# NLESC-JCER/Fortran_Davidson

Hardware: AMD Instinct MI355X
Metric: Davidson iterations/sec (dense DPR solve, matrix resident in HBM) + A*V HBM GB/s vs roofline (higher is better)
Workload: dtype f64

## Files before the change

fortran_davidson_amd/csrc/engine.hip:

```cpp
#include "engine_internal.h"

thread_local std::string g_err;
int fail(const std::string& msg) {
  g_err = msg;
  return 1;
}

int bind(E* e) {
  e->h0_take = e->h0_cols;
  e->h0_cols = 0;
  HIPCHK(hipSetDevice(e->device));
  return 0;
}

int collect_events(E* e) {
  e->ev_open = 0;
  for (int i = 0; i < e->ev_used; ++i) {
    if (!e->ev_done[i]) continue;
    HIPCHK(hipEventSynchronize(e->ev[i][1]));
    float ms = 0;
    HIPCHK(hipEventElapsedTime(&ms, e->ev[i][0], e->ev[i][1]));
    if (e->ev_kind[i] == 0) {
      e->st.apply_ms += ms;
      e->st.apply_bytes += e->ev_bytes[i];
// ... 146 lines not shown
}

Tune tune_from_env() {
  Tune t;
  auto geti = [](const char* name, int dflt) { const char* ev = getenv(name); return ev && *ev ? atoi(ev) : dflt; };
  t.sym_wide = geti("DAV_SYM_WIDE", t.sym_wide);
  t.sym_wide32 = geti("DAV_SYM_WIDE32", t.sym_wide32);
  t.sym_pair = geti("DAV_SYM_PAIR", t.sym_pair);
  t.sym_quad = geti("DAV_SYM_QUAD", t.sym_quad);
  t.sym_overlap = geti("DAV_SYM_OVERLAP", t.sym_overlap);
  t.sym_r = geti("DAV_SYM_R", t.sym_r);
  t.sym_tall = geti("DAV_SYM_TALL", t.sym_tall);
  t.sym_gen_wide = geti("DAV_SYM_GEN_WIDE", 1);
  t.sym_run = std::max(0, geti("DAV_SYM_RUN", 0));
  t.sym_run9 = std::max(0, geti("DAV_SYM_RUN9", 0));
  t.sym_mfma4 = geti("DAV_SYM_MFMA4", t.sym_mfma4);
  t.mv_target = std::max(0, geti("DAV_MV_TARGET", 0));
  t.mv_nsplit = std::max(0, geti("DAV_MV_NSPLIT", 0));
  t.b_resident = geti("DAV_B_RESIDENT", t.b_resident);
  t.coll_direct = geti("DAV_COLL_DIRECT", t.coll_direct);
  t.pg_pin = geti("DAV_PG_PIN", t.pg_pin);
  t.gram_wgs = geti("DAV_GRAM_WGS", t.gram_wgs);
  gram_set_fuse_chunks(geti("DAV_GRAM_FUSE", 0));
  t.gjd_trace = getenv("DAV_GJD_TRACE") != nullptr;
  t.harness_libm = geti("DAV_HARNESS_LIBM", 0);
  t.no_h0 = geti("DAV_NO_H0", 0);
  t.coll_select = geti("DAV_COLL_SELECT", 1);
  t.coll_trial_corrupt = geti("DAV_COLL_TRIAL_CORRUPT", 0);
  t.coll_forced = getenv("DAV_SYM_OVERLAP") != nullptr || getenv("DAV_COLL_DIRECT") != nullptr;
  return t;
// ... 456 lines not shown
```

fortran_davidson_amd/csrc/engine_apply.hip:

```cpp
#include "engine_internal.h"

bool inner_f32_tiles(E* e, OpDesc& o) {
  if (e->inner_bits != 32 || o.kind != DAV_KIND_DENSE || o.storage != 1 || o.a32_refused) return false;
  if (o.a32_valid) return true;
  const size_t count = (size_t)std::max<int64_t>(e->sym.ntiles, 1) * SYM_TB * SYM_TB;
  if (!o.a32 && pool_malloc(&o.a32, sizeof(float) * count) != hipSuccess) {
    (void)hipGetLastError();
    o.a32 = nullptr;
    o.a32_refused = true;
    return false;
  }
  launch_tiles_to_f32(e->stream, o.a, o.a32, (int64_t)count);
  o.a32_valid = true;
  return true;
}

static double* sym_slab_t(const E* e, const SymLaunch& L) { return e->sym_slab + (int64_t)L.ngroups * L.dstride; }
static void sym_sweep(E* e, const SymLaunch& L, const OpDesc& o, const SymSet& set, const double* xt) {
  if (L.nitems == 0) return;
  const SymPlan* pl = L.plan;
  const void* tiles = L.use32 ? (const void*)o.a32 : (const void*)o.a;
  double *slabD = e->sym_slab, *slabT = sym_slab_t(e, L);
  const int64_t xs = e->xt_group_stride, ds = L.dstride, ts = L.tstride;
  switch (L.family) {
    case SYM_ROW_STORED:
      return launch_matvec_sym(e->stream, o.a, set.row_off, set.items, set.nitems, xt, L.kk, slabD, slabT, L.ngroups, xs, ds, ts);
    case SYM_ROW_GENERATED:
      return launch_matvec_sym_generated(e->stream, op_params(o), e->n, set.items, set.nitems, xt, L.kk, slabD, slabT, L.ngroups, xs, ds, ts);
    case SYM_SUPER:
      return launch_matvec_sym9(e->stream, L.R, o.kind != DAV_KIND_DENSE, tiles, L.use32, set.row_off, o.kind != DAV_KIND_DENSE ? op_params(o) : OpParams{},
                                e->n, e->sym_nb, pl->items, pl->nitems, pl->zslot_begin, xt, L.kk, slabD, slabT, L.nwg, xs, ds, ts, e->tune.sym_mfma4 != 0);
    case SYM_WIDE:
    case SYM_WIDE_F32:
      return launch_matvec_symw(e->stream, L.nbw, L.tall, L.use32, tiles, set.row_off, e->sym_nb, pl->items, pl->nitems, pl->zslot_begin, xt, L.kk, slabD, slabT, L.nwg, xs, ds, ts);
    case SYM_WIDE_GENERATED:
      return launch_matvec_symw_generated(e->stream, op_params(o), e->n, e->sym_nb, pl->items, pl->nitems, pl->zslot_begin, xt, L.kk, slabD, slabT, L.nwg, xs, ds, ts);
  }
}

static void count_apply(E* e, int which, int kk) { if (which == DAV_OP_A) { e->st.applies += 1; e->st.apply_cols += kk; } }

static int pack_operand(E* e, const double* src, int kk, bool gather) {
  launch_pack_xt(e->stream, src, e->ldp, e->nloc, e->nslab, kk, e->xt, e->xt_group_stride, e->row0);
  if (!gather) return 0;
  const int ngroups = (kk + 15) / 16;
  CollGroup grp(e);
  CHK(grp.begin(5, 8.0 * (double)e->nslab * 16 * ngroups * e->nranks));
  for (int g = 0; g < ngroups; ++g)
    CHK(coll_allgather(e, e->xt + g * e->xt_group_stride + e->row0 * 16, e->xt + g * e->xt_group_stride, (size_t)e->nslab * 16));
  return grp.end("all-gather of the new block", e->stream);
}

static void sym_reduce_groups(E* e, const SymLaunch& L, const SymSet& set, const int64_t* owned, double* out, int64_t chunk_rows, bool accumulate) {
  const int64_t total_rows = (int64_t)e->nranks * e->nslab;
  const double* slabT = sym_slab_t(e, L);
  for (int g = 0; g < L.ngroups; ++g) {
    const int kg = std::min(16, L.kk - 16 * g);
    const double *d = e->sym_slab + g * L.dstride, *t = slabT + g * L.tstride;
    double* og = out + (size_t)g * 16 * (size_t)(chunk_rows ? total_rows : e->ldp);
    if (L.plan)
      launch_sym9_reduce(e->stream, d, t, L.plan->row_begin, L.plan->zslot_begin, owned, L.plan->next_owned, L.R, e->sym_nb, e->nloc, kg, og, e->ldp,
                         chunk_rows, total_rows, accumulate);
    else
      launch_sym_reduce(e->stream, d, t, set.row_begin, owned, e->sym_nb, e->nloc, kg, og, e->ldp, chunk_rows, total_rows, accumulate);
  }
}

static int ensure_sym_wpart(E* e) {
  if (e->sym_wpart) return 0;
  HIPCHK(pool_malloc(&e->sym_wpart, sizeof(double) * (size_t)e->nranks * (size_t)e->nslab * 64));
  HIPCHK(pool_malloc(&e->sym_wrecv, sizeof(double) * (size_t)e->nslab * 64));
  return 0;
}

static int sym_scatter_to_panel(E* e, int kk, double* dst, bool accumulate, const char* what, double* h0 = nullptr, size_t h0_count = 0) {
// ... 541 lines not shown
```

fortran_davidson_amd/csrc/engine_internal.h:

```cpp
#pragma once
#include "davidson_hip_private.h"
#include "kernels.h"
#include "ingest.h"

#include <dlfcn.h>
#include <fcntl.h>
#include <pthread.h>
#include <sys/mman.h>
#include <sys/stat.h>
#include <unistd.h>
#include <rccl/rccl.h>

#include <algorithm>
#include <chrono>
#include <condition_variable>
#include <ctime>
#include <mutex>
#include <cmath>
#include <cstdio>
#include <cstring>
#include <numeric>
#include <string>
#include <thread>
#include <vector>
// ... 51 lines not shown
  do {                                                                                             \
    ncclResult_t r_ = (call);                                                                      \
    if (r_ != ncclSuccess) return fail(std::string(#call) + " failed: " + g_rccl.GetErrorString(r_)); \
  } while (0)

struct LocalGroup;
struct ShmGroup;

struct SymPlan {
  int R = 0, nitems = 0, nsuper = 0;
  int64_t zslots = 0;
  int* items = nullptr;
  int* row_begin = nullptr;
  int* zslot_begin = nullptr;
  int* next_owned = nullptr;
};
struct SymSet {
  std::vector<int64_t> row_off_h;
  int64_t* row_off = nullptr;
  int64_t ntiles = 0;
  int nitems = 0;
  int* items = nullptr;
  int* row_begin = nullptr;
  SymPlan plan[2];
  bool built = false;
};
void sym_set_release(SymSet& s);
enum SymFamily { SYM_ROW_STORED, SYM_ROW_GENERATED, SYM_SUPER, SYM_WIDE, SYM_WIDE_GENERATED, SYM_WIDE_F32 };
struct SymLaunch {
  SymFamily family = SYM_SUPER;
  int kk = 0, ngroups = 0;
  int R = 0, nwg = 0, nbw = 1;
  bool use32 = false, tall = false;
  const SymPlan* plan = nullptr;
  int nitems = 0;
  int64_t dstride = 0, tstride = 0;
  int gen_evals = 0;
};

// ... 55 lines not shown

constexpr int N_SMALL = 4;
constexpr int N_EVPAIRS = 64;

struct Tune {
  int sym_wide = 2;
  int sym_wide32 = 1;
  int sym_pair = 1;
  int sym_quad = 1;
  int sym_overlap = 0;
  int sym_r = 0;
  int sym_tall = 1;
  int sym_gen_wide = 1;
  int sym_run = 0;
  int sym_run9 = 0;
  int sym_mfma4 = 1;
  int64_t mv_target = 0;
  int64_t mv_nsplit = 0;
  int gram_wgs = 0;
  int pg_pin = 1;
  int coll_direct = 0;
  int b_resident = 1;
  bool gjd_trace = false;
  int coll_select = 1;
  int coll_trial_corrupt = 0;
  bool coll_forced = false;
  int no_h0 = 0;
  int harness_libm = 0;
};
Tune tune_from_env();
// ... 220 lines not shown
```

fortran_davidson_amd/csrc/engine_operators.hip:

```cpp
#include "engine_internal.h"

int refresh_diag_host(E* e, int which) {
  if (which == DAV_OP_A) e->basis_order.clear();
  std::vector<double>& d = e->diag_host[which];
  d.assign((size_t)e->n, 0.0);
  if (!has_comm(e)) {
    CHK(need_comm(e));
    HIPCHK(hipMemcpyAsync(d.data(), e->op[which].diag, sizeof(double) * e->n, hipMemcpyDeviceToHost, e->stream));
    HIPCHK(hipStreamSynchronize(e->stream));
  } else {
    CHK(coll_allgather(e, e->op[which].diag, e->gather_dev, (size_t)e->nslab));
    HIPCHK(hipMemcpyAsync(d.data(), e->gather_dev, sizeof(double) * e->n, hipMemcpyDeviceToHost, e->stream));
    HIPCHK(hipStreamSynchronize(e->stream));
  }
  return 0;
}

static bool sym_wide_enabled(const E* e) { return e->tune.sym_wide > 1; }

static int sym_schedule(const E* e, int kk, bool stored_fp64) {
  const int forced = e->tune.sym_r;
  const int nb = (int)(e->ncols_pad / SYM_TB);
  int R = nb >= 200 ? (kk <= 8 ? 4 : 2) : (nb >= 64 && stored_fp64 ? 2 : 1);
  const bool tall = stored_fp64 && kk > 8 && kk <= 16 && nb >= 200 && sym_wide_enabled(e) && e->tune.sym_tall != 0;
// ... 9 lines not shown
  const bool stored = o.kind == DAV_KIND_DENSE;
  const int wide = e->tune.sym_wide;
  if (R == 0) {
    R = sym_schedule(e, kk, stored && !use32);
    if (use32 && R == 1) R = 2;
  }
  SymLaunch L;
  L.kk = kk; L.ngroups = L.nwg = (kk + 15) / 16; L.use32 = use32; L.R = R;
  if (R == 1) {
    L.family = stored ? SYM_ROW_STORED : SYM_ROW_GENERATED;
    L.nitems = set.nitems;
    L.dstride = (int64_t)set.nitems * 16 * SYM_TB;
    L.tstride = (int64_t)e->sym_nb * (e->sym_nb - 1) / 2 * 16 * SYM_TB;
  } else {
    L.plan = &set.plan[R == 4 ? 1 : 0];
    L.nitems = L.plan->nitems;
    L.dstride = (int64_t)L.nitems * R * 16 * SYM_TB;
    L.tstride = L.plan->zslots * 16 * SYM_TB;
    if (stored && !use32 && wide > 0 && ((R == 2 && (kk > 16 || wide > 1)) || (R == 4 && kk > 8 && kk <= 16))) {
      L.family = SYM_WIDE; L.nbw = kk > 16 ? 2 : 1; L.tall = R == 4;
    } else if (generated_polynomial(o) && R == 2 && kk > 16 && wide > 0 && e->tune.sym_gen_wide) {
      L.family = SYM_WIDE_GENERATED; L.nbw = 2;
    } else if (stored && use32 && wide > 1 && e->tune.sym_wide32 && R == 2 && kk <= 16) {
      L.family = SYM_WIDE_F32;
    }
    L.nwg = (L.ngroups + L.nbw - 1) / L.nbw;
  }
  L.gen_evals = stored ? 0 : L.nwg;
  return L;
}

std::vector<int> sym_group_owners(int nb, int nranks) {
  const int ng = (nb + 3) / 4;
  std::vector<int> owner(ng, 0);
  std::vector<int64_t> load(nranks, 0);
  for (int q = ng - 1; q >= 0; --q) {
    int64_t tiles = 0;
    for (int I = 4 * q; I < std::min(nb, 4 * q + 4); ++I) tiles += I + 1;
    int best = 0;
    for (int r = 1; r < nranks; ++r)
      if (load[r] < load[best]) best = r;
    owner[q] = best;
    load[best] += tiles;
  }
  return owner;
}

void sym_set_release(SymSet& s) {
  pool_free(s.row_off); pool_free(s.items); pool_free(s.row_begin);
  for (SymPlan& pl : s.plan) { pool_free(pl.items); pool_free(pl.row_begin); pool_free(pl.zslot_begin); pool_free(pl.next_owned); }
  s = SymSet();
}

int sym_setup(E* e) {
  if (e->sym.built) return 0;
  const int nb = (int)(e->ncols_pad / SYM_TB);
  e->sym_nb = nb;
  return sym_build_set(e, 0, nb, e->sym);
}

int sym_build_set(E* e, int first, int end, SymSet& out) {
  const int nb = (int)(e->ncols_pad / SYM_TB);
  sym_set_release(out);
  out.row_off_h.assign(nb, -1);
  int64_t ntiles = 0;
// ... 50 lines not shown
    for (const Item& it : plist) { pitems.push_back(it.I); pitems.push_back(it.J0); pitems.push_back(it.J1); pitems.push_back(it.slot); }
    pitems.resize(std::max<size_t>(pitems.size(), 4), 0);
    pl.nitems = prow[pl.nsuper];
    pl.zslots = zbeg[pl.nsuper];
    HIPCHK(pool_malloc(&pl.items, sizeof(int) * pitems.size()));
    HIPCHK(pool_malloc(&pl.row_begin, sizeof(int) * prow.size()));
    HIPCHK(pool_malloc(&pl.zslot_begin, sizeof(int) * zbeg.size()));
    HIPCHK(hipMemcpy(pl.items, pitems.data(), sizeof(int) * pitems.size(), hipMemcpyHostToDevice));
    HIPCHK(hipMemcpy(pl.row_begin, prow.data(), sizeof(int) * prow.size(), hipMemcpyHostToDevice));
    HIPCHK(hipMemcpy(pl.zslot_begin, zbeg.data(), sizeof(int) * zbeg.size(), hipMemcpyHostToDevice));
    std::vector<int> nxt(pl.nsuper + 1, pl.nsuper);
    for (int S = pl.nsuper - 1; S >= 0; --S) nxt[S] = owned(S * pl.R) ? S : nxt[S + 1];
    HIPCHK(pool_malloc(&pl.next_owned, sizeof(int) * nxt.size()));
    HIPCHK(hipMemcpy(pl.next_owned, nxt.data(), sizeof(int) * nxt.size(), hipMemcpyHostToDevice));
  }
  out.built = true;
  return 0;
}

int sym_diag(E* e, OpDesc& o) {
  if (e->nranks == 1) {
    launch_diag_sym(e->stream, o.a, e->sym.row_off, e->n, e->nloc_pad, o.diag);
    return 0;
  }
  if (!(e->comm || e->lg || e->shm)) return fail("multi-rank engine used before dav_comm_init");
  launch_diag_sym(e->stream, o.a, e->sym.row_off, e->n, e->ncols_pad, e->gather_dev);
  CHK(coll_allreduce(e, e->gather_dev, (size_t)e->ncols_pad));
  HIPCHK(hipMemcpyAsync(o.diag, e->gather_dev + e->row0, sizeof(double) * (size_t)e->nslab, hipMemcpyDeviceToDevice, e->stream));
  return 0;
}
// ... 488 lines not shown
```

fortran_davidson_amd/csrc/k_matvec_sym9.hip:

```cpp
#include "kernels.h"
#include <cstdlib>
#include <type_traits>

__device__ __forceinline__ const double* sym9_tile(const double* tiles, const int64_t* __restrict__ row_off, int I, int J) {
  return tiles + (row_off[I] + J) * (int64_t)(SYM_TB * SYM_TB);
}

__device__ __forceinline__ double mfma4_f64(double a, double b, double c) { return __builtin_amdgcn_mfma_f64_4x4x4f64(a, b, c, 0, 0, 0); }

template <int R, bool GEN, bool F32, bool M4, int HARN = 0>
__global__ __launch_bounds__(512, 1) void matvec_sym9_kernel(const void* __restrict__ tiles_v, const int64_t* __restrict__ row_off,
                                                             const int* __restrict__ items,
                                                             const int* __restrict__ zslot_begin, const double* __restrict__ xt,
                                                             double* __restrict__ slabD, double* __restrict__ slabT, int kcols,
                                                             int npair, int64_t xt_gstride, int64_t slabD_gstride,
                                                             int64_t slabT_gstride, int nb, OpParams op, int64_t n) {
  const double* tiles = static_cast<const double*>(tiles_v);
  const float* tiles32 = static_cast<const float*>(tiles_v);
  (void)tiles; (void)tiles32;
  constexpr int NCG = 4 / R;
  constexpr int NRS = 2 * R;
  constexpr int BW = 16 * NCG;
  constexpr int UPJ = SYM_TB / BW;
  constexpr int UPS = 64 / BW;
// ... 388 lines not shown
  const int64_t row = (int64_t)J * SYM_TB + r;
  if (chunk_rows > 0) {
    if (row < total_rows) dst[(row / chunk_rows) * (chunk_rows * k) + (int64_t)col * chunk_rows + row % chunk_rows] = sum;
  } else {
    dst[(int64_t)col * ldd + row] = row < nloc ? (accumulate ? dst[(int64_t)col * ldd + row] + sum : sum) : 0.0;
  }
}

void launch_sym9_reduce(hipStream_t st, const double* slabD, const double* slabT, const int* row_item_begin_dev,
                        const int* zslot_begin_dev, const int64_t* owned, const int* next_owned, int R, int nb, int64_t nloc, int k, double* dst,
                        int64_t ldd, int64_t chunk_rows, int64_t total_rows, bool accumulate) {
  const int nsuper = (nb + R - 1) / R;
  hipLaunchKernelGGL(sym9_reduce_kernel, dim3(nb, k), dim3(256), 0, st, slabD, slabT, row_item_begin_dev, zslot_begin_dev, owned, next_owned, R,
                     nb, nsuper, nloc, k, dst, ldd, chunk_rows, total_rows, accumulate && chunk_rows == 0 ? 1 : 0);
}
```

fortran_davidson_amd/csrc/k_matvec_symw.hip:

```cpp
#include "kernels.h"
#include <cstdlib>
#include <type_traits>
#include <utility>

#define MFMA_DRAIN "s_nop 15\n\ts_nop 3"

typedef int i32x4 __attribute__((ext_vector_type(4)));

template <class F, int... Is>
__device__ __forceinline__ void symw_static_for_impl(F&& f, std::integer_sequence<int, Is...>) { (f(std::integral_constant<int, Is>{}), ...); }
template <int N, class F>
__device__ __forceinline__ void symw_static_for(F&& f) { symw_static_for_impl(f, std::make_integer_sequence<int, N>{}); }

#define SYMW_RING(k, u) (224 - 16 * NSLOT + 16 * (k) + 4 * (u))
#define SYMW_XJ(s, u, bcb) (224 + 16 * (s) + 4 * (u) + 2 * (bcb))
#define SYMW_P(par, ib, j) (SYMW_PBASE + 16 * (par) + 8 * (ib) + 4 * (j))
#define SYMW_RAW(k, u) (224 + 8 * (k) + 2 * (u))
#ifndef SYMW_HARN_GROUP
#define SYMW_HARN_GROUP 1
#endif
#define SYMW_LROW(hs) (200 + 4 * (hs))
#define SYMW_LCOL(u) (216 + 2 * (u))
constexpr int symw_fixed_lo(bool harness) { return harness ? 168 : 128; }

// ... 4 lines not shown
#define STAMP(t) do { __builtin_amdgcn_sched_barrier(0); asm volatile("s_memtime %0\n\ts_waitcnt lgkmcnt(0)" : "=s"(t) :: "memory"); __builtin_amdgcn_sched_barrier(0); } while (0)
extern "C" int dav_symw_stamps(unsigned long long* out) {
  unsigned long long z[12] = {0, 0, 0, 0, 0, 0, 0, 0, 0, 0, 0, 0};
  if (hipMemcpyFromSymbol(out, HIP_SYMBOL(symw_stamp), sizeof(z)) != hipSuccess) return 1;
  return hipMemcpyToSymbol(HIP_SYMBOL(symw_stamp), z, sizeof(z)) != hipSuccess;
}
#else
#define STAMP(t) do { } while (0)
#endif

__device__ __forceinline__ unsigned symw_uniform(unsigned x) { return (unsigned)__builtin_amdgcn_readfirstlane((int)x); }
__device__ __forceinline__ int64_t symw_uniform(int64_t x) {
  const uint64_t u = (uint64_t)x;
  return (int64_t)(((uint64_t)symw_uniform((unsigned)(u >> 32)) << 32) | symw_uniform((unsigned)u));
}
__device__ __forceinline__ const char* symw_uniform(const char* p) { return reinterpret_cast<const char*>(symw_uniform((int64_t)reinterpret_cast<uintptr_t>(p))); }

__device__ __forceinline__ i32x4 symw_desc(const void* p, int bytes) {
  const uint64_t a = reinterpret_cast<uint64_t>(p);
  return i32x4{(int)symw_uniform((unsigned)a), (int)symw_uniform((unsigned)(a >> 32) & 0xffffu), bytes, 0x00020000};
}

template <int NB, bool TALL, bool F32, int GEN>
__global__ __launch_bounds__(256, 1) void matvec_symw_kernel(const void* __restrict__ tiles_any, const int64_t* __restrict__ row_off,
                                                             const int* __restrict__ items, const int* __restrict__ zslot_begin,
                                                             const double* __restrict__ xt, double* __restrict__ slabD,
                                                             double* __restrict__ slabT, int kcols, int nwg, int64_t xt_gstride,
                                                             int64_t slabD_gstride, int64_t slabT_gstride, int nb, OpParams op, int64_t n) {
  static_assert(!TALL || NB == 1, "two slices per wave: 16 columns per workgroup");
  static_assert(GEN == 0 || (NB == 2 && !TALL && !F32), "generated entries: 32 columns, two block rows per workgroup");
  constexpr bool HARN = GEN >= 2;
  constexpr int SYMW_PBASE = symw_fixed_lo(HARN);
  constexpr bool REGT = F32 || GEN != 0;
  (void)op; (void)n;
  static_assert(!F32 || (NB == 1 && !TALL), "fp32 tiles: 16 columns, two block rows per workgroup");
  using TileT = std::conditional_t<F32, float, double>;
  const TileT* __restrict__ tiles = static_cast<const TileT*>(tiles_any);
  constexpr int R = TALL ? 4 : 2;
  constexpr int NSL = TALL ? 2 : 1;
  constexpr int NRS = 4;
  constexpr unsigned UPJ = SYM_TB / 16;
// ... 19 lines not shown
      item = nfull / nwg + (blockIdx.x - nfull) / nwg;
      grp = (blockIdx.x - nfull) % nwg;
    }
  } else {
    item = blockIdx.x;
    grp = 0;
  }
  xt += (int64_t)grp * NB * xt_gstride;
  slabD += (int64_t)grp * NB * slabD_gstride;
  slabT += (int64_t)grp * NB * slabT_gstride;
  kcols -= 16 * NB * grp;

  const unsigned lane = threadIdx.x & 63;
  const int wave = __builtin_amdgcn_readfirstlane(threadIdx.x >> 6);
  const unsigned c = lane & 15, g = lane >> 4;
  const int S = items[4 * item], J0 = items[4 * item + 1], J1 = items[4 * item + 2];
  const int I0 = S * R;
  const int Imax = I0 + R - 1 < nb - 1 ? I0 + R - 1 : nb - 1;
  const int rhalf = wave & 1;
  int Is[NSL];
  bool have_row[NSL];
#pragma unroll
  for (int sl = 0; sl < NSL; ++sl) { Is[sl] = I0 + 2 * sl + (wave >> 1); have_row[sl] = Is[sl] <= Imax; }

  double xI[NSL][4][2][2][2][NB];
#pragma unroll
  for (int sl = 0; sl < NSL; ++sl) {
    const double* xr = xt + ((int64_t)(have_row[sl] ? Is[sl] : Imax) * SYM_TB + 128 * rhalf) * 16;
    const unsigned xo = (4 * g) * 16 + c;
#pragma unroll
    for (int hs = 0; hs < 4; ++hs)
// ... 211 lines not shown
    constexpr int SLOT = decltype(slot)::value;
    symw_static_for<4>([&](auto uc) {
      constexpr int U = decltype(uc)::value;
      double x, y;
      asm volatile("v_cvt_f64_f32 %0, v%c2\n\tv_cvt_f64_f32 %1, v%c3" : "=&v"(x), "=&v"(y) : "i"(SYMW_RAW(SLOT, U)), "i"(SYMW_RAW(SLOT, U) + 1));
      w[U] = f64x2{x, y};
    });
  };
  auto ds_r = [&](auto parc, auto tc) {
    constexpr int PAR = decltype(parc)::value, IB = decltype(tc)::value >> 1, JJ = decltype(tc)::value & 1;
    const unsigned ra = tw_rd;
    asm volatile("ds_read_b128 a[%c1:%c2], %0 offset:%c3"
                 :: "v"(ra), "i"(SYMW_P(PAR, IB, JJ)), "i"(SYMW_P(PAR, IB, JJ) + 3), "i"((16 * IB + 2 * JJ) * (int)sizeof(double)) : "memory");
  };

  const int64_t zbase = zslot_begin[S];
  unsigned qz[R];
#pragma unroll
  for (int r = 0; r < R; ++r) qz[r] = symw_uniform(I0 + r <= Imax && I0 + r > J0 ? (unsigned)(I0 + r - J0) * UPJ : 0u);
  unsigned zoff[NB];
#pragma unroll
  for (int t = 0; t < NB; ++t) {
    const unsigned e = wave * (NB * 64) + 64 * t + lane;
    const unsigned bcb = e >> 8, half = (e >> 7) & 1, ln = (e & 127) >> 1, jj = e & 1;
    zoff[t] = (16 * bcb + (ln & 15)) * ZS + (ln >> 4) + 4 * (2 * half + jj);
  }
  unsigned long long st_hs = 0, st_bar = 0, st_sum = 0, st_unit = 0, st_vm = 0, st_mf = 0;
  (void)st_hs; (void)st_bar; (void)st_sum; (void)st_unit; (void)st_vm; (void)st_mf;
#ifdef DAV_SYMW_STAMPS
  unsigned long long tk0, tr0;
  asm volatile("s_memtime %0\n\ts_memrealtime %1\n\ts_waitcnt lgkmcnt(0)" : "=s"(tk0), "=s"(tr0) :: "memory");
// ... 18 lines not shown
    const int un = w / (2 * NB), bcb = (w / 2) % NB, half = w & 1;
    double* zr = &zred[pair & 1][wave][un][0];
    *reinterpret_cast<f64x2*>(zr + 256 * bcb + 128 * half + 2 * lane) = f64x2{z[un][bcb][2 * half], z[un][bcb][2 * half + 1]};
  };
  auto flush_strip = [&](unsigned st) {
    const int J = J0 + (int)(st >> 2);
    if (J >= Imax) return;
    const double* zs = zst[st & 1];
#pragma unroll
    for (int bcb = 0; bcb < NB; ++bcb) {
      const int kc = kcols - 16 * bcb < 16 ? kcols - 16 * bcb : 16;
      double* outT = slabT + bcb * slabT_gstride + (zbase + J) * 16 * SYM_TB + (st & 3) * ZW;
#pragma unroll
      for (int h = 0; h < 2; ++h) {
        const int e = threadIdx.x + 256 * h, bc = e >> 5, pr = e & 31;
        if (bc < kc) *reinterpret_cast<f64x2*>(outT + bc * SYM_TB + 2 * pr) = *reinterpret_cast<const f64x2*>(zs + (16 * bcb + bc) * ZS + 2 * pr);
      }
    }
  };

  static_assert(DEPTH == 3 && NSLOT == 4, "the counts below hold for a 4-slot ring with 3 half-steps of lookahead");
  constexpr auto younger = [](int hs) { return 4 + (NBL / 2) * (hs == 0 ? 0 : hs == 2 ? 2 : 1); };
  i32x4 ud[3];
  if constexpr (GEN == 0) { ud[0] = unit_desc(0); ud[1] = unit_desc(1); ud[2] = unit_desc(2); }
  symw_static_for<NB>([&](auto bc) {
    const i32x4 d = x_desc(0, decltype(bc)::value);
    symw_static_for<4>([&](auto uc) { x_load(std::integral_constant<int, 0>{}, uc, bc, d, std::true_type{}); });
  });
  if constexpr (GEN == 0) {
    symw_static_for<DEPTH>([&](auto sc) {
      constexpr int st = decltype(sc)::value;
// ... 193 lines not shown
    for (int t = 0; t < NB; ++t) sum_finish(nseq - un, t);
  }
  __syncthreads();
  flush_strip(nunits / UPS - 1);
#ifdef DAV_SYMW_STAMPS
  if (lane == 0) {
    unsigned long long tk1, tr1;
    asm volatile("s_memtime %0\n\ts_memrealtime %1\n\ts_waitcnt lgkmcnt(0)" : "=s"(tk1), "=s"(tr1) :: "memory");
    atomicAdd(&symw_stamp[0], st_hs); atomicAdd(&symw_stamp[1], st_bar); atomicAdd(&symw_stamp[2], st_sum);
    atomicAdd(&symw_stamp[3], (unsigned long long)nunits);
    atomicAdd(&symw_stamp[4], tk1 - tk0); atomicAdd(&symw_stamp[5], tr1 - tr0); atomicAdd(&symw_stamp[6], st_vm); atomicAdd(&symw_stamp[9], st_mf);
    atomicAdd(&symw_stamp[10], st_unit); atomicAdd(&symw_stamp[11], 1ull);
  }
#endif

  double* outD = slabD + (int64_t)items[4 * item + 3] * R * 16 * SYM_TB;
#pragma unroll
  for (int sl = 0; sl < NSL; ++sl) {
#pragma unroll
    for (int bcb = 0; bcb < NB; ++bcb) {
      const int kc = kcols - 16 * bcb < 16 ? kcols - 16 * bcb : 16;
#pragma unroll
      for (int hs = 0; hs < 4; ++hs) {
        asm volatile(MFMA_DRAIN : "+v"(acc[sl][hs][0][bcb]), "+v"(acc[sl][hs][1][bcb]));
#pragma unroll
        for (int par = 0; par < 2; ++par)
#pragma unroll
          for (int reg = 0; reg < 4; ++reg) tw[c * RS + 2 * (g + 4 * reg) + par] = acc[sl][hs][par][bcb][reg];
#pragma unroll
        for (int t = 0; t < 8; ++t) {
          const int e = lane + 64 * t;
          const int bc = e >> 5, r = e & 31;
          const double v = tw[bc * RS + r];
          if (bc < kc && have_row[sl])
            outD[bcb * slabD_gstride + ((int64_t)(2 * sl + (wave >> 1)) * 16 + bc) * SYM_TB + 128 * rhalf + 32 * hs + r] = v;
        }
      }
    }
  }
  asm volatile("" ::: "a128", "a255");
  if constexpr (F32) asm volatile("" ::: "v224", "v255");
}

void launch_matvec_symw(hipStream_t st, int nbw, bool tall, bool tiles_f32, const void* tiles, const int64_t* row_off, int nb, const int* items_dev,
                        int nitems, const int* zslot_begin_dev, const double* xt, int kcols, double* slabD, double* slabT, int nwg,
                        int64_t xt_gstride, int64_t slabD_gstride, int64_t slabT_gstride) {
  dim3 grid(nitems * nwg), block(256);
  const OpParams op{};
  const int64_t n = 0;
#define SYMW_LAUNCH(NBW, T, F)                                                                                                          \
  hipLaunchKernelGGL((matvec_symw_kernel<NBW, T, F, 0>), grid, block, 0, st, tiles, row_off, items_dev, zslot_begin_dev, xt, slabD, slabT, kcols, \
                     nwg, xt_gstride, slabD_gstride, slabT_gstride, nb, op, n)
  if (tiles_f32) SYMW_LAUNCH(1, false, true);
  else if (nbw == 2) SYMW_LAUNCH(2, false, false);
  else if (tall) SYMW_LAUNCH(1, true, false);
  else SYMW_LAUNCH(1, false, false);
#undef SYMW_LAUNCH
}

void launch_matvec_symw_generated(hipStream_t st, OpParams op, int64_t n, int nb, const int* items_dev, int nitems, const int* zslot_begin_dev,
                                  const double* xt, int kcols, double* slabD, double* slabT, int nwg, int64_t xt_gstride, int64_t slabD_gstride,
                                  int64_t slabT_gstride) {
#define SYMW_GEN_LAUNCH(G)                                                                                                                       \
  hipLaunchKernelGGL((matvec_symw_kernel<2, false, false, G>), dim3(nitems * nwg), dim3(256), 0, st, (const void*)nullptr, (const int64_t*)nullptr, \
                     items_dev, zslot_begin_dev, xt, slabD, slabT, kcols, nwg, xt_gstride, slabD_gstride, slabT_gstride, nb, op, n)
  if (op.kind == DAV_KIND_HARNESS) { if (op.trig != 0) SYMW_GEN_LAUNCH(3); else SYMW_GEN_LAUNCH(2); }
  else SYMW_GEN_LAUNCH(1);
#undef SYMW_GEN_LAUNCH
}
```

fortran_davidson_amd/csrc/kernels.h:

```cpp
#pragma once
#include "common.h"

constexpr int MV_ROWS = 256;
void launch_pack_xt(hipStream_t st, const double* src, int64_t ld, int64_t nloc, int64_t nslab, int k,
                    double* xt, int64_t xt_group_stride, int64_t row_off);
void launch_matvec_dense(hipStream_t st, const double* A, int64_t lda, int64_t nrows_pad, int64_t ncols_pad,
                         const double* xt, int64_t xt_group_stride, int ngroups, double* slab,
                         int nsplit, int jc);
void launch_matvec_free(hipStream_t st, OpParams op, int64_t row0, int64_t nloc, int64_t n,
                        int64_t nrows_pad, int64_t ncols_pad, const double* xt, int64_t xt_group_stride,
                        int ngroups, double* slab, int nsplit, int jc);
void launch_slab_reduce(hipStream_t st, const double* slab, int nsplit, int64_t nrows_pad, int ngroups,
                        int64_t nloc, int k, double* dst, int64_t ldd);
size_t matvec_slab_doubles(int64_t nrows_pad, int ngroups, int nsplit);
void matvec_plan(int64_t nrows_pad, int64_t ncols_pad, int ngroups, int* nsplit, int* jc, int64_t target = 0, int64_t forced_nsplit = 0);

constexpr int GRAM_MIN_ROWS = 256;
constexpr int GRAM_FUSE_CHUNKS = 24;
constexpr int GRAM_MAX_COUNTERS = 256;
void launch_gram(hipStream_t st, const double* P, int64_t ldp, int p, const double* Q, int64_t ldq, int q,
                 int64_t nrows_pad, double* scratch, double* out_dev, unsigned* counters = nullptr, int wg_target = 0);
size_t gram_scratch_doubles(int p, int q, int64_t nrows_pad);
void gram_set_fuse_chunks(int n);
void launch_gram_multi(hipStream_t st, const double* P, int64_t ldp, int p, const double* const* Qs, int nq, int qeach, int64_t ldq,
// ... 55 lines not shown
int coldots_blocks(int64_t nrows_pad);
void launch_coldots(hipStream_t st, const DotsArgs& a);

constexpr int SYM_TB = 256;
void launch_matvec_sym(hipStream_t st, const double* tiles, const int64_t* row_off, const int* items_dev, int nitems, const double* xt, int kcols,
                       double* slabD, double* slabT, int npair, int64_t xt_gstride, int64_t slabD_gstride, int64_t slabT_gstride);
void launch_matvec_sym_generated(hipStream_t st, OpParams op, int64_t n, const int* items_dev, int nitems, const double* xt, int kcols,
                                 double* slabD, double* slabT, int npair, int64_t xt_gstride, int64_t slabD_gstride,
                                 int64_t slabT_gstride);
void launch_sym_reduce(hipStream_t st, const double* slabD, const double* slabT, const int* row_item_begin_dev, const int64_t* owned,
                       int nb, int64_t nloc, int k, double* dst, int64_t ldd, int64_t chunk_rows, int64_t total_rows, bool accumulate = false);
void launch_matvec_sym9(hipStream_t st, int R, bool gen, const void* tiles, bool tiles_f32, const int64_t* row_off, OpParams op, int64_t n,
                        int nb, const int* items_dev, int nitems, const int* zslot_begin_dev, const double* xt, int kcols, double* slabD,
                        double* slabT, int npair, int64_t xt_gstride, int64_t slabD_gstride, int64_t slabT_gstride, bool mfma4 = true);
void launch_matvec_symw(hipStream_t st, int nbw, bool tall, bool tiles_f32, const void* tiles, const int64_t* row_off, int nb, const int* items_dev,
                        int nitems, const int* zslot_begin_dev, const double* xt, int kcols, double* slabD, double* slabT, int nwg,
                        int64_t xt_gstride, int64_t slabD_gstride, int64_t slabT_gstride);
void launch_matvec_symw_generated(hipStream_t st, OpParams op, int64_t n, int nb, const int* items_dev, int nitems, const int* zslot_begin_dev,
                                  const double* xt, int kcols, double* slabD, double* slabT, int nwg, int64_t xt_gstride, int64_t slabD_gstride,
                                  int64_t slabT_gstride);
void launch_tiles_to_f32(hipStream_t st, const double* src, float* dst, int64_t count);
void launch_sym9_reduce(hipStream_t st, const double* slabD, const double* slabT, const int* row_item_begin_dev,
                        const int* zslot_begin_dev, const int64_t* owned, const int* next_owned, int R, int nb, int64_t nloc, int k, double* dst,
                        int64_t ldd, int64_t chunk_rows, int64_t total_rows, bool accumulate = false);
void launch_generate_sym_tiles(hipStream_t st, double* tiles, const int64_t* row_off_host, int nb, int64_t n, uint64_t seed,
                               double sparsity, int use_diag, double diag_val);
void launch_retile_panel(hipStream_t st, const double* panel, int64_t ldp, int64_t nrows, int ncols, int J, int nb,
                         const int64_t* row_off, double* tiles);
void launch_diag_sym(hipStream_t st, const double* tiles, const int64_t* row_off, int64_t n, int64_t nrows, double* diag);
void launch_gather_columns_sym_rs(hipStream_t st, const double* tiles, const int64_t* row_off, int64_t n, int64_t chunk_rows,
                                  int64_t total_rows, const int64_t* idx_dev, int k, double* dst);
void launch_entries_sym(hipStream_t st, const double* tiles, const int64_t* row_off, const int64_t* idx_dev, int k, double* h0);
void launch_zero_pad_rows(hipStream_t st, double* dst, int64_t ldd, int64_t nloc, int64_t nrows_pad, int k);
void launch_entries_free(hipStream_t st, OpParams op, const int64_t* idx_dev, int k, double* h0);
void launch_entries_dense(hipStream_t st, const double* A, int64_t lda, const int64_t* idx_dev, int k, double* h0);
void launch_gather_columns_free(hipStream_t st, OpParams op, int64_t row0, int64_t nloc, int64_t nrows_pad, const int64_t* idx_dev, int k,
                                double* dst, int64_t ldd);
void launch_gather_columns_sym(hipStream_t st, const double* tiles, const int64_t* row_off, int64_t n, int64_t nrows_pad,
                               const int64_t* idx_dev, int k, double* dst, int64_t ldd);
// ... 85 lines not shown
```

Baseline: 23.62.

## Chain adjacent super-rows in wide symmetric matvec to reuse transposed strips

Adds a chained work plan for the R=2, two-block-wide stored symmetric matvec. One workgroup processes several consecutive super-rows that share a column range, and members after the first accumulate their transposed contributions into a shared strip with f64 atomics. A new indexed reduce kernel gathers the diagonal and transposed partials per block row. The aim is to cut transposed-slab storage and the reduce traffic, and to balance items by sorting them by work. In exchange it adds atomic adds, __syncthreads between members, and a gather-based reduce.

```diff
diff --git a/fortran_davidson_amd/csrc/engine.hip b/fortran_davidson_amd/csrc/engine.hip
--- a/fortran_davidson_amd/csrc/engine.hip
+++ b/fortran_davidson_amd/csrc/engine.hip
@@ -184,6 +184,9 @@
   t.sym_gen_wide = geti("DAV_SYM_GEN_WIDE", 1);
   t.sym_run = std::max(0, geti("DAV_SYM_RUN", 0));
   t.sym_run9 = std::max(0, geti("DAV_SYM_RUN9", 0));
+  t.sym_chain = std::max(1, geti("DAV_SYM_CHAIN", t.sym_chain));
+  t.sym_chain_run = std::max(1, geti("DAV_SYM_CHAIN_RUN", t.sym_chain_run));
+  t.sym_chain_low = std::max(0, geti("DAV_SYM_CHAIN_LOW", t.sym_chain_low));
   t.sym_mfma4 = geti("DAV_SYM_MFMA4", t.sym_mfma4);
   t.mv_target = std::max(0, geti("DAV_MV_TARGET", 0));
   t.mv_nsplit = std::max(0, geti("DAV_MV_NSPLIT", 0));
diff --git a/fortran_davidson_amd/csrc/engine_apply.hip b/fortran_davidson_amd/csrc/engine_apply.hip
--- a/fortran_davidson_amd/csrc/engine_apply.hip
+++ b/fortran_davidson_amd/csrc/engine_apply.hip
@@ -32,7 +32,7 @@
                                 e->n, e->sym_nb, pl->items, pl->nitems, pl->zslot_begin, xt, L.kk, slabD, slabT, L.nwg, xs, ds, ts, e->tune.sym_mfma4 != 0);
     case SYM_WIDE:
     case SYM_WIDE_F32:
-      return launch_matvec_symw(e->stream, L.nbw, L.tall, L.use32, tiles, set.row_off, e->sym_nb, pl->items, pl->nitems, pl->zslot_begin, xt, L.kk, slabD, slabT, L.nwg, xs, ds, ts);
+      return launch_matvec_symw(e->stream, L.nbw, L.tall, L.use32, tiles, set.row_off, e->sym_nb, pl->items, pl->nitems, pl->zslot_begin, pl->chain, xt, L.kk, slabD, slabT, L.nwg, xs, ds, ts);
     case SYM_WIDE_GENERATED:
       return launch_matvec_symw_generated(e->stream, op_params(o), e->n, e->sym_nb, pl->items, pl->nitems, pl->zslot_begin, xt, L.kk, slabD, slabT, L.nwg, xs, ds, ts);
   }
@@ -58,7 +58,9 @@
     const int kg = std::min(16, L.kk - 16 * g);
     const double *d = e->sym_slab + g * L.dstride, *t = slabT + g * L.tstride;
     double* og = out + (size_t)g * 16 * (size_t)(chunk_rows ? total_rows : e->ldp);
-    if (L.plan)
+    if (L.plan && L.plan->chain)
+      launch_sym_chain_reduce(e->stream, d, t, L.plan->red_off, L.plan->red_idx, e->sym_nb, e->nloc, kg, og, e->ldp, chunk_rows, total_rows, accumulate);
+    else if (L.plan)
       launch_sym9_reduce(e->stream, d, t, L.plan->row_begin, L.plan->zslot_begin, owned, L.plan->next_owned, L.R, e->sym_nb, e->nloc, kg, og, e->ldp,
                          chunk_rows, total_rows, accumulate);
     else
diff --git a/fortran_davidson_amd/csrc/engine_internal.h b/fortran_davidson_amd/csrc/engine_internal.h
--- a/fortran_davidson_amd/csrc/engine_internal.h
+++ b/fortran_davidson_amd/csrc/engine_internal.h
@@ -89,6 +89,10 @@
   int* row_begin = nullptr;
   int* zslot_begin = nullptr;
   int* next_owned = nullptr;
+  int64_t dslots = 0;
+  int* chain = nullptr;
+  int* red_off = nullptr;
+  int* red_idx = nullptr;
 };
 struct SymSet {
   std::vector<int64_t> row_off_h;
@@ -97,7 +101,7 @@
   int nitems = 0;
   int* items = nullptr;
   int* row_begin = nullptr;
-  SymPlan plan[2];
+  SymPlan plan[3];
   bool built = false;
 };
 void sym_set_release(SymSet& s);
@@ -183,6 +187,9 @@
   int sym_gen_wide = 1;
   int sym_run = 0;
   int sym_run9 = 0;
+  int sym_chain = 4;
+  int sym_chain_run = 16;
+  int sym_chain_low = 120;
   int sym_mfma4 = 1;
   int64_t mv_target = 0;
   int64_t mv_nsplit = 0;
diff --git a/fortran_davidson_amd/csrc/engine_operators.hip b/fortran_davidson_amd/csrc/engine_operators.hip
--- a/fortran_davidson_amd/csrc/engine_operators.hip
+++ b/fortran_davidson_amd/csrc/engine_operators.hip
@@ -1,4 +1,5 @@
 #include "engine_internal.h"
+#include "sym_chain_plan.h"
 
 int refresh_diag_host(E* e, int which) {
   if (which == DAV_OP_A) e->basis_order.clear();
@@ -47,9 +48,6 @@
     L.tstride = (int64_t)e->sym_nb * (e->sym_nb - 1) / 2 * 16 * SYM_TB;
   } else {
     L.plan = &set.plan[R == 4 ? 1 : 0];
-    L.nitems = L.plan->nitems;
-    L.dstride = (int64_t)L.nitems * R * 16 * SYM_TB;
-    L.tstride = L.plan->zslots * 16 * SYM_TB;
     if (stored && !use32 && wide > 0 && ((R == 2 && (kk > 16 || wide > 1)) || (R == 4 && kk > 8 && kk <= 16))) {
       L.family = SYM_WIDE; L.nbw = kk > 16 ? 2 : 1; L.tall = R == 4;
     } else if (generated_polynomial(o) && R == 2 && kk > 16 && wide > 0 && e->tune.sym_gen_wide) {
@@ -57,6 +55,10 @@
     } else if (stored && use32 && wide > 1 && e->tune.sym_wide32 && R == 2 && kk <= 16) {
       L.family = SYM_WIDE_F32;
     }
+    if (L.family == SYM_WIDE && L.nbw == 2 && R == 2 && set.plan[2].chain) L.plan = &set.plan[2];
+    L.nitems = L.plan->nitems;
+    L.dstride = (L.plan->chain ? L.plan->dslots : (int64_t)L.nitems) * R * 16 * SYM_TB;
+    L.tstride = L.plan->zslots * 16 * SYM_TB;
     L.nwg = (L.ngroups + L.nbw - 1) / L.nbw;
   }
   L.gen_evals = stored ? 0 : L.nwg;
@@ -81,7 +83,10 @@
 
 void sym_set_release(SymSet& s) {
   pool_free(s.row_off); pool_free(s.items); pool_free(s.row_begin);
-  for (SymPlan& pl : s.plan) { pool_free(pl.items); pool_free(pl.row_begin); pool_free(pl.zslot_begin); pool_free(pl.next_owned); }
+  for (SymPlan& pl : s.plan) {
+    pool_free(pl.items); pool_free(pl.row_begin); pool_free(pl.zslot_begin); pool_free(pl.next_owned);
+    pool_free(pl.chain); pool_free(pl.red_off); pool_free(pl.red_idx);
+  }
   s = SymSet();
 }
 
@@ -162,6 +167,25 @@
     HIPCHK(pool_malloc(&pl.next_owned, sizeof(int) * nxt.size()));
     HIPCHK(hipMemcpy(pl.next_owned, nxt.data(), sizeof(int) * nxt.size(), hipMemcpyHostToDevice));
   }
+  if (e->tune.sym_chain > 1 && e->nranks == 1 && first == 0 && ntiles == (int64_t)nb * (nb + 1) / 2) {
+    SymPlan& pl = out.plan[2];
+    int64_t Cp = std::min<int64_t>(32, std::max<int64_t>(1, (ntiles + 3071) / (3072 * 2)));
+    if (e->tune.sym_run9 > 0) Cp = e->tune.sym_run9;
+    const SymChainPlan cp = sym_chain_plan(nb, e->tune.sym_chain, e->tune.sym_chain_run, (int)Cp, e->tune.sym_chain_low);
+    pl.R = 2;
+    pl.nsuper = (nb + 1) / 2;
+    pl.nitems = cp.nitems;
+    pl.dslots = cp.dslots;
+    pl.zslots = cp.zslots;
+    HIPCHK(pool_malloc(&pl.items, sizeof(int) * cp.items.size()));
+    HIPCHK(pool_malloc(&pl.chain, sizeof(int) * cp.chain.size()));
+    HIPCHK(pool_malloc(&pl.red_off, sizeof(int) * cp.red_off.size()));
+    HIPCHK(pool_malloc(&pl.red_idx, sizeof(int) * std::max<size_t>(cp.red_idx.size(), 1)));
+    HIPCHK(hipMemcpy(pl.items, cp.items.data(), sizeof(int) * cp.items.size(), hipMemcpyHostToDevice));
+    HIPCHK(hipMemcpy(pl.chain, cp.chain.data(), sizeof(int) * cp.chain.size(), hipMemcpyHostToDevice));
+    HIPCHK(hipMemcpy(pl.red_off, cp.red_off.data(), sizeof(int) * cp.red_off.size(), hipMemcpyHostToDevice));
+    if (!cp.red_idx.empty()) HIPCHK(hipMemcpy(pl.red_idx, cp.red_idx.data(), sizeof(int) * cp.red_idx.size(), hipMemcpyHostToDevice));
+  }
   out.built = true;
   return 0;
 }
diff --git a/fortran_davidson_amd/csrc/k_matvec_sym9.hip b/fortran_davidson_amd/csrc/k_matvec_sym9.hip
--- a/fortran_davidson_amd/csrc/k_matvec_sym9.hip
+++ b/fortran_davidson_amd/csrc/k_matvec_sym9.hip
@@ -426,3 +426,32 @@
   hipLaunchKernelGGL(sym9_reduce_kernel, dim3(nb, k), dim3(256), 0, st, slabD, slabT, row_item_begin_dev, zslot_begin_dev, owned, next_owned, R,
                      nb, nsuper, nloc, k, dst, ldd, chunk_rows, total_rows, accumulate && chunk_rows == 0 ? 1 : 0);
 }
+
+__global__ __launch_bounds__(256) void sym_chain_reduce_kernel(const double* __restrict__ slabD, const double* __restrict__ slabT,
+                                                               const int* __restrict__ red_off, const int* __restrict__ red_idx, int64_t nloc,
+                                                               int k, double* __restrict__ dst, int64_t ldd, int64_t chunk_rows,
+                                                               int64_t total_rows, int accumulate) {
+  const int J = blockIdx.x, col = blockIdx.y, r = threadIdx.x;
+  if (col >= k) return;
+  const int d0 = red_off[2 * J], t0 = red_off[2 * J + 1], t1 = red_off[2 * J + 2];
+  double sum = 0.0;
+  for (int i = d0; i < t0; ++i) sum += slabD[((int64_t)red_idx[i] * 16 + col) * SYM_TB + r];
+  auto zt = [&](int i) { return slabT[((int64_t)red_idx[i] * 16 + col) * SYM_TB + r]; };
+  double s0 = 0.0, s1 = 0.0, s2 = 0.0, s3 = 0.0;
+  int i = t0;
+  for (; i + 3 < t1; i += 4) { s0 += zt(i); s1 += zt(i + 1); s2 += zt(i + 2); s3 += zt(i + 3); }
+  for (; i < t1; ++i) s0 += zt(i);
+  sum += (s0 + s1) + (s2 + s3);
+  const int64_t row = (int64_t)J * SYM_TB + r;
+  if (chunk_rows > 0) {
+    if (row < total_rows) dst[(row / chunk_rows) * (chunk_rows * k) + (int64_t)col * chunk_rows + row % chunk_rows] = sum;
+  } else {
+    dst[(int64_t)col * ldd + row] = row < nloc ? (accumulate ? dst[(int64_t)col * ldd + row] + sum : sum) : 0.0;
+  }
+}
+
+void launch_sym_chain_reduce(hipStream_t st, const double* slabD, const double* slabT, const int* red_off_dev, const int* red_idx_dev, int nb,
+                             int64_t nloc, int k, double* dst, int64_t ldd, int64_t chunk_rows, int64_t total_rows, bool accumulate) {
+  hipLaunchKernelGGL(sym_chain_reduce_kernel, dim3(nb, k), dim3(256), 0, st, slabD, slabT, red_off_dev, red_idx_dev, nloc, k, dst, ldd, chunk_rows,
+                     total_rows, accumulate && chunk_rows == 0 ? 1 : 0);
+}
diff --git a/fortran_davidson_amd/csrc/k_matvec_symw.hip b/fortran_davidson_amd/csrc/k_matvec_symw.hip
--- a/fortran_davidson_amd/csrc/k_matvec_symw.hip
+++ b/fortran_davidson_amd/csrc/k_matvec_symw.hip
@@ -42,6 +42,9 @@
   const uint64_t u = (uint64_t)x;
   return (int64_t)(((uint64_t)symw_uniform((unsigned)(u >> 32)) << 32) | symw_uniform((unsigned)u));
 }
+__device__ __forceinline__ void symw_add_f64(double* p, double v) {
+  (void)__builtin_amdgcn_global_atomic_fadd_f64(reinterpret_cast<__attribute__((address_space(1))) double*>(reinterpret_cast<uintptr_t>(p)), v);
+}
 __device__ __forceinline__ const char* symw_uniform(const char* p) { return reinterpret_cast<const char*>(symw_uniform((int64_t)reinterpret_cast<uintptr_t>(p))); }
 
 __device__ __forceinline__ i32x4 symw_desc(const void* p, int bytes) {
@@ -52,7 +55,7 @@
 template <int NB, bool TALL, bool F32, int GEN>
 __global__ __launch_bounds__(256, 1) void matvec_symw_kernel(const void* __restrict__ tiles_any, const int64_t* __restrict__ row_off,
                                                              const int* __restrict__ items, const int* __restrict__ zslot_begin,
-                                                             const double* __restrict__ xt, double* __restrict__ slabD,
+                                                             const int* __restrict__ chain, const double* __restrict__ xt, double* __restrict__ slabD,
                                                              double* __restrict__ slabT, int kcols, int nwg, int64_t xt_gstride,
                                                              int64_t slabD_gstride, int64_t slabT_gstride, int nb, OpParams op, int64_t n) {
   static_assert(!TALL || NB == 1, "two slices per wave: 16 columns per workgroup");
@@ -102,7 +105,14 @@
   const unsigned lane = threadIdx.x & 63;
   const int wave = __builtin_amdgcn_readfirstlane(threadIdx.x >> 6);
   const unsigned c = lane & 15, g = lane >> 4;
-  const int S = items[4 * item], J0 = items[4 * item + 1], J1 = items[4 * item + 2];
+  const int J0 = items[4 * item + 1], J1 = items[4 * item + 2];
+  constexpr bool CHAINS = NB == 2 && !TALL && !F32 && GEN == 0;
+  const bool chained = CHAINS && chain != nullptr;
+  const int members = chained ? __builtin_amdgcn_readfirstlane(chain[2 * item]) : 1;
+  const int64_t zbase = chained ? chain[2 * item + 1] : zslot_begin[items[4 * item]];
+#pragma nounroll
+  for (int member = 0; member < members; ++member) {
+  const int S = items[4 * item] + member;
   const int I0 = S * R;
   const int Imax = I0 + R - 1 < nb - 1 ? I0 + R - 1 : nb - 1;
   const int rhalf = wave & 1;
@@ -344,7 +354,6 @@
                  :: "v"(ra), "i"(SYMW_P(PAR, IB, JJ)), "i"(SYMW_P(PAR, IB, JJ) + 3), "i"((16 * IB + 2 * JJ) * (int)sizeof(double)) : "memory");
   };
 
-  const int64_t zbase = zslot_begin[S];
   unsigned qz[R];
 #pragma unroll
   for (int r = 0; r < R; ++r) qz[r] = symw_uniform(I0 + r <= Imax && I0 + r > J0 ? (unsigned)(I0 + r - J0) * UPJ : 0u);
@@ -393,7 +402,15 @@
 #pragma unroll
       for (int h = 0; h < 2; ++h) {
         const int e = threadIdx.x + 256 * h, bc = e >> 5, pr = e & 31;
-        if (bc < kc) *reinterpret_cast<f64x2*>(outT + bc * SYM_TB + 2 * pr) = *reinterpret_cast<const f64x2*>(zs + (16 * bcb + bc) * ZS + 2 * pr);
+        if (bc < kc) {
+          const f64x2 v = *reinterpret_cast<const f64x2*>(zs + (16 * bcb + bc) * ZS + 2 * pr);
+          double* o = outT + bc * SYM_TB + 2 * pr;
+          if (!CHAINS || member == 0) *reinterpret_cast<f64x2*>(o) = v;
+          else {
+            symw_add_f64(o, v.x);
+            symw_add_f64(o + 1, v.y);
+          }
+        }
       }
     }
   };
@@ -617,7 +634,7 @@
   }
 #endif
 
-  double* outD = slabD + (int64_t)items[4 * item + 3] * R * 16 * SYM_TB;
+  double* outD = slabD + (int64_t)(items[4 * item + 3] + member) * R * 16 * SYM_TB;
 #pragma unroll
   for (int sl = 0; sl < NSL; ++sl) {
 #pragma unroll
@@ -641,18 +658,20 @@
       }
     }
   }
+  if (CHAINS && member + 1 < members) __syncthreads();
+  }
   asm volatile("" ::: "a128", "a255");
   if constexpr (F32) asm volatile("" ::: "v224", "v255");
 }
 
 void launch_matvec_symw(hipStream_t st, int nbw, bool tall, bool tiles_f32, const void* tiles, const int64_t* row_off, int nb, const int* items_dev,
-                        int nitems, const int* zslot_begin_dev, const double* xt, int kcols, double* slabD, double* slabT, int nwg,
+                        int nitems, const int* zslot_begin_dev, const int* chain_dev, const double* xt, int kcols, double* slabD, double* slabT, int nwg,
                         int64_t xt_gstride, int64_t slabD_gstride, int64_t slabT_gstride) {
   dim3 grid(nitems * nwg), block(256);
   const OpParams op{};
   const int64_t n = 0;
 #define SYMW_LAUNCH(NBW, T, F)                                                                                                          \
-  hipLaunchKernelGGL((matvec_symw_kernel<NBW, T, F, 0>), grid, block, 0, st, tiles, row_off, items_dev, zslot_begin_dev, xt, slabD, slabT, kcols, \
+  hipLaunchKernelGGL((matvec_symw_kernel<NBW, T, F, 0>), grid, block, 0, st, tiles, row_off, items_dev, zslot_begin_dev, chain_dev, xt, slabD, slabT, kcols, \
                      nwg, xt_gstride, slabD_gstride, slabT_gstride, nb, op, n)
   if (tiles_f32) SYMW_LAUNCH(1, false, true);
   else if (nbw == 2) SYMW_LAUNCH(2, false, false);
@@ -666,7 +685,7 @@
                                   int64_t slabT_gstride) {
 #define SYMW_GEN_LAUNCH(G)                                                                                                                       \
   hipLaunchKernelGGL((matvec_symw_kernel<2, false, false, G>), dim3(nitems * nwg), dim3(256), 0, st, (const void*)nullptr, (const int64_t*)nullptr, \
-                     items_dev, zslot_begin_dev, xt, slabD, slabT, kcols, nwg, xt_gstride, slabD_gstride, slabT_gstride, nb, op, n)
+                     items_dev, zslot_begin_dev, (const int*)nullptr, xt, slabD, slabT, kcols, nwg, xt_gstride, slabD_gstride, slabT_gstride, nb, op, n)
   if (op.kind == DAV_KIND_HARNESS) { if (op.trig != 0) SYMW_GEN_LAUNCH(3); else SYMW_GEN_LAUNCH(2); }
   else SYMW_GEN_LAUNCH(1);
 #undef SYMW_GEN_LAUNCH
diff --git a/fortran_davidson_amd/csrc/kernels.h b/fortran_davidson_amd/csrc/kernels.h
--- a/fortran_davidson_amd/csrc/kernels.h
+++ b/fortran_davidson_amd/csrc/kernels.h
@@ -93,7 +93,7 @@
                         int nb, const int* items_dev, int nitems, const int* zslot_begin_dev, const double* xt, int kcols, double* slabD,
                         double* slabT, int npair, int64_t xt_gstride, int64_t slabD_gstride, int64_t slabT_gstride, bool mfma4 = true);
 void launch_matvec_symw(hipStream_t st, int nbw, bool tall, bool tiles_f32, const void* tiles, const int64_t* row_off, int nb, const int* items_dev,
-                        int nitems, const int* zslot_begin_dev, const double* xt, int kcols, double* slabD, double* slabT, int nwg,
+                        int nitems, const int* zslot_begin_dev, const int* chain_dev, const double* xt, int kcols, double* slabD, double* slabT, int nwg,
                         int64_t xt_gstride, int64_t slabD_gstride, int64_t slabT_gstride);
 void launch_matvec_symw_generated(hipStream_t st, OpParams op, int64_t n, int nb, const int* items_dev, int nitems, const int* zslot_begin_dev,
                                   const double* xt, int kcols, double* slabD, double* slabT, int nwg, int64_t xt_gstride, int64_t slabD_gstride,
@@ -102,6 +102,8 @@
 void launch_sym9_reduce(hipStream_t st, const double* slabD, const double* slabT, const int* row_item_begin_dev,
                         const int* zslot_begin_dev, const int64_t* owned, const int* next_owned, int R, int nb, int64_t nloc, int k, double* dst,
                         int64_t ldd, int64_t chunk_rows, int64_t total_rows, bool accumulate = false);
+void launch_sym_chain_reduce(hipStream_t st, const double* slabD, const double* slabT, const int* red_off_dev, const int* red_idx_dev, int nb,
+                             int64_t nloc, int k, double* dst, int64_t ldd, int64_t chunk_rows, int64_t total_rows, bool accumulate = false);
 void launch_generate_sym_tiles(hipStream_t st, double* tiles, const int64_t* row_off_host, int nb, int64_t n, uint64_t seed,
                                double sparsity, int use_diag, double diag_val);
 void launch_retile_panel(hipStream_t st, const double* panel, int64_t ldp, int64_t nrows, int ncols, int J, int nb,
diff --git a/fortran_davidson_amd/csrc/sym_chain_plan.h b/fortran_davidson_amd/csrc/sym_chain_plan.h
--- /dev/null
+++ b/fortran_davidson_amd/csrc/sym_chain_plan.h
@@ -0,0 +1,77 @@
+#pragma once
+#include <algorithm>
+#include <cstdint>
+#include <vector>
+
+struct SymChainPlan {
+  int nitems = 0;
+  int64_t dslots = 0, zslots = 0;
+  std::vector<int> items;
+  std::vector<int> chain;
+  std::vector<int> red_off, red_idx;
+};
+
+inline SymChainPlan sym_chain_plan(int nb, int c, int run_chained, int run_single, int low) {
+  SymChainPlan P;
+  const int R = 2, nsuper = (nb + R - 1) / R;
+  run_chained = std::max(1, run_chained);
+  run_single = std::max(1, run_single);
+  low = std::max(low, 1);
+  std::vector<int> first(nsuper, -1);
+  if (c > 1)
+    for (int hi = nb / R; hi - c >= low; hi -= c)
+      for (int S = hi - c; S < hi; ++S) first[S] = hi - c;
+  struct Item { int S, J0, J1, slot, members, zbase; };
+  struct Strip { int zbase, Jlo, Jhi; };
+  std::vector<Item> list;
+  std::vector<Strip> strips;
+  int dslot = 0, zslot = 0;
+  auto cut = [&](int S, int Jlo, int Jhi, int run, int members, int zbase) {
+    for (int J0 = Jlo; J0 < Jhi; J0 += run) {
+      list.push_back({S, J0, std::min(Jhi, J0 + run), dslot, members, zbase});
+      dslot += members;
+    }
+  };
+  for (int S = 0; S < nsuper; ++S) {
+    const int Imax = std::min(S * R + R - 1, nb - 1);
+    int Jlo = 0;
+    if (first[S] >= 0) {
+      Jlo = R * first[S];
+      if (first[S] == S) {
+        cut(S, 0, Jlo, run_chained, c, zslot);
+        strips.push_back({zslot, 0, Jlo});
+        zslot += Jlo;
+      }
+    }
+    cut(S, Jlo, Imax + 1, run_single, 1, zslot - Jlo);
+    if (Imax > Jlo) strips.push_back({zslot - Jlo, Jlo, Imax});
+    zslot += Imax - Jlo;
+  }
+  P.nitems = (int)list.size();
+  P.dslots = dslot;
+  P.zslots = zslot;
+  std::vector<std::vector<int>> dl(nb), tl(nb);
+  for (const Item& it : list)
+    for (int m = 0; m < it.members; ++m)
+      for (int sub = 0; sub < R; ++sub)
+        if ((it.S + m) * R + sub < nb) dl[(it.S + m) * R + sub].push_back((it.slot + m) * R + sub);
+  for (const Strip& s : strips)
+    for (int J = s.Jlo; J < s.Jhi; ++J) tl[J].push_back(s.zbase + J);
+  P.red_off.assign(2 * nb + 1, 0);
+  for (int J = 0; J < nb; ++J) {
+    P.red_off[2 * J] = (int)P.red_idx.size();
+    P.red_idx.insert(P.red_idx.end(), dl[J].begin(), dl[J].end());
+    P.red_off[2 * J + 1] = (int)P.red_idx.size();
+    P.red_idx.insert(P.red_idx.end(), tl[J].begin(), tl[J].end());
+  }
+  P.red_off[2 * nb] = (int)P.red_idx.size();
+  std::stable_sort(list.begin(), list.end(),
+                   [](const Item& a, const Item& b) { return a.members * (a.J1 - a.J0) > b.members * (b.J1 - b.J0); });
+  for (const Item& it : list) {
+    P.items.insert(P.items.end(), {it.S, it.J0, it.J1, it.slot});
+    P.chain.insert(P.chain.end(), {it.members, it.zbase});
+  }
+  P.items.resize(std::max<size_t>(P.items.size(), 4), 0);
+  P.chain.resize(std::max<size_t>(P.chain.size(), 2), 1);
+  return P;
+}
```

Result: no change. 23.83 (median of 6 runs) (+0.9%).
